# sapienta-ai/general-motion-retargeting

Measured on AMD Instinct MI355X. Metric: retargeted frames/sec (whole node) + max joint-angle err vs CPU ref, G1 29-DoF, higher is better.
Workload: dtype f64

## Files before the change

general_motion_retargeting_amd/csrc/gmr_ik.hip:

```cpp
#include <hip/hip_runtime.h>
#include <math.h>
#include <stdint.h>

#include "../../include/gmr_hip.h"
#include "gmr_device_math.h"
#include "gmr_ik_layout.h"
#include "gmr_ik_prof.h"

namespace gmr {

template <int NW>
__device__ __forceinline__ void wsync() {
  if (NW == 1) __syncthreads();
  else __builtin_amdgcn_fence(__ATOMIC_SEQ_CST, "workgroup");
}
#define WSYNC() wsync<NW>()

#ifndef GMR_IK_MIN_WAVES
#define GMR_IK_MIN_WAVES 1
#endif
enum { QP_DENSE = 0, QP_TREE_SMALL = 1, QP_TREE = 2 };
enum { CMD_BUILD = 1, CMD_EXIT = 2, CMD_JBODY = 3 };

__device__ __forceinline__ double readlane_d(double v, int src) {
  int lo = __builtin_amdgcn_readlane(__double2loint(v), src);
  int hi = __builtin_amdgcn_readlane(__double2hiint(v), src);
  return __hiloint2double(hi, lo);
}

__device__ __forceinline__ double bpermute_d(int addr, double v) {
  int lo = __builtin_amdgcn_ds_bpermute(addr, __double2loint(v));
  int hi = __builtin_amdgcn_ds_bpermute(addr, __double2hiint(v));
  return __hiloint2double(hi, lo);
}

__device__ __forceinline__ double dot6(const double* a, const double* b) {
  return a[0] * b[0] + a[1] * b[1] + a[2] * b[2] + a[3] * b[3] + a[4] * b[4] + a[5] * b[5];
}

}
#include "gmr_ik_tree.h"
namespace gmr {

struct FkLane {
  int dep, hinge, src[IK_MAX_HOPS];
  d4 bq; d3 bp, ax;
};

template <class LT>
__device__ __forceinline__ FkLane fk_lane(const LT& L, const double* sm, const short* hop, const short* depth,
                                          const short* body_hinge, int lane) {
  FkLane F;
  const int b = lane < L.nb ? lane : 0;
  F.dep = lane < L.nb ? depth[b] : 0;
  F.hinge = lane < L.nb ? body_hinge[b] : -1;
#pragma unroll
  for (int r = 0; r < IK_MAX_HOPS; r++) F.src[r] = r < L.nhop ? 4 * hop[r * L.o.cap.nb + b] : 0;
  const double* bq = sm + L.o.body_quat + 4 * b;
  const double* bp = sm + L.o.body_pos + 3 * b;
  const double* ax = sm + L.o.axis + 3 * b;
  F.bq = d4{bq[0], bq[1], bq[2], bq[3]};
  F.bp = d3{bp[0], bp[1], bp[2]};
  F.ax = d3{ax[0], ax[1], ax[2]};
  return F;
}

template <int NW, class LT>
__device__ __forceinline__ void fk_wave(const LT& L, double* sm, const FkLane& F, int lane, Prof& pr) {
  lane = fresh_lane(lane);
  PROF_BEGIN(pr);
  const int nb = L.nb;
  double* q = sm + L.o.q;
  d3 pos = {0, 0, 0};
  d4 quat = {1, 0, 0, 0};
  const int dep = F.dep;
  if (lane < nb) {
    if (lane == 0) {
      quat = qnormalize(d4{q[3], q[4], q[5], q[6]});
      q[3] = quat.w; q[4] = quat.x; q[5] = quat.y; q[6] = quat.z;
      pos = d3{q[0], q[1], q[2]};
    } else {
      quat = F.bq;
      pos = F.bp;
      if (F.hinge >= 0) {
        const double* sc = sm + L.o.hsc + 2 * F.hinge;
        const double s = sc[0], c = sc[1];
        quat = qmul(quat, d4{c, F.ax.x * s, F.ax.y * s, F.ax.z * s});
      }
    }
  }
#pragma unroll
  for (int r = 0; r < IK_MAX_HOPS; r++) {
    if (r >= L.nhop) break;
    const int src = F.src[r];
    const d3 pa = {bpermute_d(src, pos.x), bpermute_d(src, pos.y), bpermute_d(src, pos.z)};
    const d4 qa = {bpermute_d(src, quat.w), bpermute_d(src, quat.x), bpermute_d(src, quat.y), bpermute_d(src, quat.z)};
    if (NW > 1) __builtin_amdgcn_s_waitcnt(0xc07f);
    if (lane < nb && dep >= (1 << r)) {
      pos = pa + qrot(qa, pos);
      quat = qmul(qa, quat);
    }
  }
  if (lane < nb) {
    quat = qnormalize(quat);
    double* o = sm + L.o.xa + 7 * lane;
    o[0] = pos.x; o[1] = pos.y; o[2] = pos.z; o[3] = quat.w; o[4] = quat.x; o[5] = quat.y; o[6] = quat.z;
    if (F.hinge >= 0) {
      d3 aw = qrot(quat, F.ax);
      double* xa = sm + L.o.xaxis + 3 * lane;
      xa[0] = aw.x; xa[1] = aw.y; xa[2] = aw.z;
    }
  }
  WSYNC();
  PROF_END(pr, PH_FK);
}

template <int NW, class LT>
__device__ __forceinline__ double errors_wave(const LT& L, double* sm, const short* task_body,
                                              const short* task_human, int K, int lane, Prof& pr) {
  lane = fresh_lane(lane);
  PROF_BEGIN(pr);
  double ss = 0.0;
  if (lane < K) {
    int b = task_body[lane], h = task_human[lane];
    const double* x = sm + L.o.xa + 7 * b;
    const double* tg = sm + L.o.tgt + 7 * h;
    double e[6], aux[5];
    se3_log_rel5(d3{x[0], x[1], x[2]}, d4{x[3], x[4], x[5], x[6]}, d3{tg[0], tg[1], tg[2]},
                 d4{tg[3], tg[4], tg[5], tg[6]}, e, aux);
    double* eo = sm + L.o.e + 6 * lane;
#pragma unroll
    for (int r = 0; r < 6; r++) { eo[r] = e[r]; ss += e[r] * e[r]; }
    double* ao = sm + L.o.eaux + 5 * lane;
#pragma unroll
    for (int r = 0; r < 5; r++) ao[r] = aux[r];
  }
  ss = row0_sum(ss);
  WSYNC();
  PROF_END(pr, PH_ERR);
  return sqrt(ss);
}

struct StageTabs {
  const short* task_body; const short* task_human; const short* pair_task; const short* pair_dof;
  const short* pair_index; const uint2* items;
};

template <int NW, class LT>
__device__ __forceinline__ double jlog_phase(const LT& L, double* sm, int stage, double lm_damping, int lane,
                                             Prof& pr) {
  lane = fresh_lane(lane);
  PROF_BEGIN(pr);
  const int K = L.K[stage];
  const double* wpos = sm + L.o.wpos[stage];
  const double* wrot = sm + L.o.wrot[stage];
  double mu = 0.0;
  const int k = lane & 15, j = lane >> 4;
  if (NW > 1) {
    if (lane < K) {
      const double* e = sm + L.o.e + 6 * lane;
      double ee[6];
#pragma unroll
      for (int r = 0; r < 6; r++) ee[r] = e[r];
      const double* ax = sm + L.o.eaux + 5 * lane;
      const double aux[5] = {ax[0], ax[1], ax[2], ax[3], ax[4]};
      double coef[8];
      se3_jlinv_coef5(ee, aux, coef);
      double* co = sm + L.o.M + 18 * lane;
#pragma unroll
      for (int r = 0; r < 8; r++) co[r] = coef[r];
      const double wp = wpos[lane], wr = wrot[lane];
      double* we = sm + L.o.we + 6 * lane;
#pragma unroll
      for (int r = 0; r < 6; r++) {
        double v = (r < 3 ? wp : wr) * ee[r];
        we[r] = v;
        mu += v * v;
      }
    }
  } else if (k < K && j < 3) {
    const double* e = sm + L.o.e + 6 * k;
    double ee[6];
#pragma unroll
    for (int r = 0; r < 6; r++) ee[r] = e[r];
    const double* ax = sm + L.o.eaux + 5 * k;
    const double aux[5] = {ax[0], ax[1], ax[2], ax[3], ax[4]};
    double Ac[3], Bc[3];
    se3_jlinv_col5(ee, aux, j, Ac, Bc);
    double* M = sm + L.o.M + 18 * k + j;
#pragma unroll
    for (int i = 0; i < 3; i++) { M[3 * i] = -Ac[i]; M[9 + 3 * i] = -Bc[i]; }
    if (j == 0) {
      double wp = wpos[k], wr = wrot[k];
      double* we = sm + L.o.we + 6 * k;
#pragma unroll
      for (int r = 0; r < 6; r++) {
        double v = (r < 3 ? wp : wr) * ee[r];
        we[r] = v;
        mu += v * v;
      }
    }
  }
  mu = lm_damping * row0_sum(mu);
  WSYNC();
  PROF_END(pr, PH_JLOG);
  return mu;
}

template <class LT>
__device__ __forceinline__ void pairs_phase(const LT& L, double* sm, int stage, const StageTabs& tb,
                                            const short* hinge_body, int vlane, int nvl) {
  const int P = L.P[stage];
  const double* wpos = sm + L.o.wpos[stage];
  const double* wrot = sm + L.o.wrot[stage];
  double* Jw = sm + L.o.Jw;
  double* cpart = sm + L.o.cpart;
  const double* X = sm + L.o.xa;
  for (int p = vlane; p < P; p += nvl) {
    const unsigned info = (unsigned short)tb.pair_task[p];
    const int k = info & 15u, dof = (info >> 4) & 63u, b = info >> 10;
    const int c = tb.pair_dof[p];
    d3 pb = {X[7 * b], X[7 * b + 1], X[7 * b + 2]};
    d4 qb = {X[7 * b + 3], X[7 * b + 4], X[7 * b + 5], X[7 * b + 6]};
    d3 lin, ang;
    if (dof < 3) {
      lin = d3{dof == 0 ? 1.0 : 0.0, dof == 1 ? 1.0 : 0.0, dof == 2 ? 1.0 : 0.0};
      ang = d3{0.0, 0.0, 0.0};
    } else if (dof < 6) {
      d4 q0 = {X[3], X[4], X[5], X[6]};
      int a = dof - 3;
      ang = qrot(q0, d3{a == 0 ? 1.0 : 0.0, a == 1 ? 1.0 : 0.0, a == 2 ? 1.0 : 0.0});
      lin = cross(ang, pb - d3{X[0], X[1], X[2]});
    } else {
// ... 290 lines not shown
    PROF_END(hp, PH_CVEC);
    PROF_BEGIN(hp);
    hacc_phase(L, sm, stage, tb, diag, (wave - 1) * 64 + lane, first);
    PROF_END(hp, PH_HACC);
    PROF_BEGIN(hp);
    __syncthreads();
    PROF_END(hp, PH_JLOG);
    if (QP == QP_TREE_SMALL) (void)solve_qp_tree<7, 9, false, true>(L, sm, const_cast<uint32_t*>(sw), si, wave, lane, bs, hp, rows_s);
    else (void)solve_qp_tree<8, 10, false, false>(L, sm, const_cast<uint32_t*>(sw), si, wave, lane, bs, hp, rows_l);
  }
}

template <int NVP, int NW, class LT>
__device__ __forceinline__ int solve_qp_regs(const LT& L, double* sm, int lane, int& st, Prof& pr) {
  constexpr int LDK = NVP + 1;
  const int n = L.nv, ldh = L.o.ldh;
  const double* H = sm + L.o.H;
  double* Kt = sm + L.o.Kt;
  const bool act = lane < n;
  const bool row = lane < NVP;
  const double lo = act ? (sm + L.o.lo)[lane] : 0.0, hi = act ? (sm + L.o.hi)[lane] : 0.0;
  const double ci = act ? (sm + L.o.c)[lane] : 0.0;
  const double* Hrow = H + (act ? lane : 0) * ldh;
  if (!act || (st < 0 && !(lo > -INFINITY)) || (st > 0 && !(hi < INFINITY))) st = 0;
  const double dual_tol = 1e-13 * (1.0 + rows3_max(fabs(ci)));
  const double ptol_lo = 1e-12 * (1.0 + fabs(lo)), ptol_hi = 1e-12 * (1.0 + fabs(hi));
  int pcount = 3, ninf_best = NVP + 1;
  for (int it = 0; it < 100; it++) {
    PROF_BEGIN(pr);
    PROF_COUNT(pr, PH_NFACT);
    const unsigned long long fixedm = __ballot(act && st != 0);
    const double xfix = st < 0 ? lo : (st > 0 ? hi : 0.0);
    double rhs = act ? (st != 0 ? xfix : -ci) : 0.0;
    {
      unsigned long long m = fixedm;
      while (m) {
        int j = __ffsll((long long)m) - 1;
        m &= m - 1;
        double xj = readlane_d(xfix, j);
        if (act && st == 0) rhs -= Hrow[j] * xj;
      }
    }
    const bool self_fixed = (st != 0) || !act;
    double r[NVP];
#pragma unroll
    for (int k = 0; k < NVP; k++) {
      const bool kfixed = (k >= n) || ((fixedm >> k) & 1ull);
      double h = (act && k < n && k <= lane) ? Hrow[k] : 0.0;
      double v = (self_fixed || kfixed) ? 0.0 : h;
      if (k == lane && self_fixed) v = 1.0;
      r[k] = v;
    }
    PROF_END(pr, PH_KBUILD);
    PROF_BEGIN(pr);
    double mydinv = 1.0;
    bool bad = false;
#pragma unroll
    for (int j = 0; j < NVP; j++) {
      double dj = readlane_d(r[j], j);
      bad = bad || !(dj > 0.0);
      double dinv = fast_rsqrt(dj);
      double l = r[j] * dinv;
      r[j] = l;
      if (lane == j) mydinv = dinv;
#pragma unroll
      for (int k0 = j + 1; k0 < NVP; k0 += 4) {
        double lk[4];
#pragma unroll
        for (int u = 0; u < 4; u++) lk[u] = (k0 + u < NVP) ? readlane_d(l, k0 + u) : 0.0;
        __builtin_amdgcn_sched_barrier(0);
#pragma unroll
        for (int u = 0; u < 4; u++)
          if (k0 + u < NVP) r[k0 + u] = fma(-l, lk[u], r[k0 + u]);
        __builtin_amdgcn_sched_barrier(0);
      }
    }
    if (bad) return GMR_STATUS_QP_FAILED;
    PROF_END(pr, PH_CHOL);
    PROF_BEGIN(pr);
    double b = rhs;
#pragma unroll
    for (int j = 0; j < NVP; j++) {
      double yj = readlane_d(b * mydinv, j);
      double upd = fma(-r[j], yj, b);
      b = lane == j ? yj : (lane > j ? upd : b);
    }
    if (row) {
#pragma unroll
      for (int k = 0; k < NVP; k++) Kt[lane * LDK + k] = r[k];
    }
    WSYNC();
    double lt[NVP];
#pragma unroll
    for (int j = 0; j < NVP; j++) lt[j] = row ? Kt[j * LDK + lane] : 0.0;
#pragma unroll
    for (int j = NVP - 1; j >= 0; j--) {
      double xj = readlane_d(b * mydinv, j);
      double upd = fma(-lt[j], xj, b);
      b = lane == j ? xj : (lane < j ? upd : b);
    }
    double x = b;
    WSYNC();
    PROF_END(pr, PH_SUBST);
    PROF_BEGIN(pr);
    double g = 0.0;
    if (fixedm) {
      g = ci;
#pragma unroll
      for (int j = 0; j < NVP; j++) {
        double xj = readlane_d(x, j);
        if (j < n) g += (act ? Hrow[j] : 0.0) * xj;
      }
    }
    int newst = st;
    bool viol = false;
    if (act) {
      if (st == 0) {
        if (x < lo - ptol_lo) { viol = true; newst = -1; }
        else if (x > hi + ptol_hi) { viol = true; newst = 1; }
      } else if (st < 0) {
        if (g < -dual_tol) { viol = true; newst = 0; }
      } else {
        if (g > dual_tol) { viol = true; newst = 0; }
      }
    }
    const unsigned long long vm = __ballot(viol);
    PROF_END(pr, PH_MULT);
    if (vm == 0ull) {
      if (act) (sm + L.o.x)[lane] = fmin(fmax(x, lo), hi);
      WSYNC();
      return GMR_STATUS_OK;
    }
    const int ninf = __popcll(vm);
    if (ninf < ninf_best) { ninf_best = ninf; pcount = 3; st = newst; }
    else if (pcount > 0) { pcount--; st = newst; }
    else {
      int top = 63 - __clzll((long long)vm);
      if (lane == top) st = newst;
    }
  }
  return GMR_STATUS_QP_MAXITER;
}

template <class LT>
__device__ __forceinline__ void hinge_sincos(const LT& L, double* sm, int lane) {
  if (lane >= 6 && lane < L.nv) {
    double s, c;
    sincos_small(0.5 * (sm + L.o.q)[7 + lane - 6], &s, &c);
    double* sc = sm + L.o.hsc + 2 * (lane - 6);
    sc[0] = s; sc[1] = c;
  }
}

template <int NW, class LT>
__device__ __forceinline__ void integrate_wave(const LT& L, double* sm, double dt, int lane, Prof& pr) {
  lane = fresh_lane(lane);
  PROF_BEGIN(pr);
  double* q = sm + L.o.q;
  const double* dq = sm + L.o.x;
  const bool base = lane == 0, hinge = lane >= 6 && lane < L.nv;
  double half = 0.0, inv = 0.0;
  bool rotate = false;
  if (base) {
    q[0] += dq[0]; q[1] += dq[1]; q[2] += dq[2];
    const double n2 = dq[3] * dq[3] + dq[4] * dq[4] + dq[5] * dq[5];
    rotate = n2 >= 1e-30 * dt * dt;
    if (rotate) { inv = fast_rsqrt(n2); half = 0.5 * (n2 * inv); }
  } else if (hinge) {
    const double th = q[7 + lane - 6] + dq[lane];
    q[7 + lane - 6] = th;
    half = 0.5 * th;
  }
  double s, c;
  sincos_small(half, &s, &c);
  if (base) {
    d4 quat = qnormalize(d4{q[3], q[4], q[5], q[6]});
    if (rotate) quat = qmul(quat, d4{c, dq[3] * inv * s, dq[4] * inv * s, dq[5] * inv * s});
    q[3] = quat.w; q[4] = quat.x; q[5] = quat.y; q[6] = quat.z;
  } else if (hinge) {
    double* sc = sm + L.o.hsc + 2 * (lane - 6);
    sc[0] = s; sc[1] = c;
  }
  WSYNC();
  PROF_END(pr, PH_INTEG);
}

template <int NW, class LT>
__device__ __forceinline__ void preprocess_wave(const LT& L, double* sm, const short* is_foot, int human_root,
                                                double ground_offset, int flags, int lane, Prof& pr) {
  lane = fresh_lane(lane);
  PROF_BEGIN(pr);
  const double* raw = sm + L.o.raw;
  double* tgt = sm + L.o.tgt;
  double z = INFINITY;
  d3 p = {0, 0, 0};
  d4 uq = {1, 0, 0, 0};
  const bool on = lane < L.nhum;
  if (on) {
    const double* in = raw + 7 * lane;
    const double* rp = raw + 7 * human_root;
    const double* sc = sm + L.o.scale;
    double sr = sc[human_root];
    d3 srp = {sr * rp[0], sr * rp[1], sr * rp[2]};
    if (lane == human_root) p = srp;
    else {
      double s = sc[lane];
      p = d3{(in[0] - rp[0]) * s + srp.x, (in[1] - rp[1]) * s + srp.y, (in[2] - rp[2]) * s + srp.z};
    }
    const double* qo = sm + L.o.quat_off + 4 * lane;
    const double* po = sm + L.o.pos_off + 3 * lane;
    d4 q = qnormalize(d4{in[3], in[4], in[5], in[6]});
    uq = qnormalize(qmul(q, qnormalize(d4{qo[0], qo[1], qo[2], qo[3]})));
    p = p + qrot(uq, d3{po[0], po[1], po[2]});
    if (is_foot[lane] && p.x == p.x) z = p.z;
  }
  if (flags & GMR_FLAG_OFFSET_TO_GROUND) {
    double lowest = row0_min(z);
    p.z = p.z - lowest + ground_offset;
  }
  if (on) {
    double* o = tgt + 7 * lane;
    o[0] = p.x; o[1] = p.y; o[2] = p.z; o[3] = uq.w; o[4] = uq.x; o[5] = uq.y; o[6] = uq.z;
  }
  WSYNC();
  PROF_END(pr, PH_PRE);
}

template <int NVP, int NW, int QP>
__global__ __launch_bounds__(64 * NW, GMR_IK_MIN_WAVES) void ik_streams_kernel(const uint4* __restrict__ image, IkLay<NVP, NW> L, IkParams P,
                                                             int S, int T, const double* __restrict__ q0,
                                                             const double* __restrict__ human,
                                                             const int32_t* __restrict__ len, int flags,
                                                             double* __restrict__ q_out,
                                                             int32_t* __restrict__ nsolve,
                                                             int32_t* __restrict__ status,
                                                             double* __restrict__ tgt_out,
                                                             double* __restrict__ err_out,
                                                             unsigned long long* __restrict__ prof_out) {
  extern __shared__ __align__(16) double smem[];
  const int wave = threadIdx.x >> 6;
  const int lane = threadIdx.x & 63;
  const int s = blockIdx.x;
  if (s >= S) return;
  double* sm = smem;
  Prof pr;
#ifdef GMR_IK_PROFILE
  for (int i = 0; i < PH_COUNT; i++) pr.acc[i] = 0;
  const unsigned long long k_t0 = __builtin_amdgcn_s_memtime(), k_r0 = __builtin_amdgcn_s_memrealtime();
#endif
  short* si = reinterpret_cast<short*>(smem + L.o.n_double);
  uint32_t* sw = reinterpret_cast<uint32_t*>(si + L.o.n_short);
  int* ctl = reinterpret_cast<int*>(sw + L.o.w_ctl);
  short* hop = si + L.o.i_hop;
  short* depth = si + L.o.i_depth;
  short* body_hinge = si + L.o.i_body_hinge;
  short* hinge_body = si + L.o.i_hinge_body;
  short* limited = si + L.o.i_limited;
  short* is_foot = si + L.o.i_is_foot;

  const int nv = L.nv, nq = L.nq, nhum = L.nhum;
  {
    uint4* dst = reinterpret_cast<uint4*>(smem);
    const int n16 = (L.smem_bytes + 15) >> 4;
    for (int i = threadIdx.x; i < n16; i += 64 * NW) dst[i] = image[i];
  }
  __syncthreads();
  if (NW > 1 && wave > 0) {
    helper_loop<NW, QP>(L, sm, sw, si, hinge_body, ctl, wave, lane, pr);
#ifdef GMR_IK_PROFILE
    if (wave == 1 && lane == 0 && prof_out)
      for (int i = 0; i < PH_COUNT; i++) prof_out[((size_t)S + s) * PH_COUNT + i] = pr.acc[i];
#endif
    return;
  }
  const double* prm = sm + L.o.params;
  const int max_iter = P.max_iter, human_root = P.human_root;
  const int use0 = P.use0, use1 = P.use1;

  for (int i = lane; i < nq; i += 64) (sm + L.o.q)[i] = q0[(size_t)s * nq + i];
  WSYNC();
  hinge_sincos(L, sm, lane);
  WSYNC();
  const FkLane fkc = fk_lane(L, sm, hop, depth, body_hinge, lane);
  int pk_main[2];
#pragma unroll
  for (int st = 0; st < 2; st++) pk_main[st] = (unsigned short)(si + L.o.i_pair_task[st])[lane] & 15u;
  fk_wave<NW>(L, sm, fkc, lane, pr);

  const int Ts = len ? min(len[s], T) : T;
  const size_t fstride = (size_t)nhum * 7;
  const double* hs = human + (size_t)s * T * fstride;
  int stat = GMR_STATUS_OK;
  int qp_state = 0;
  TreeState tree_state = {0ull, 0ull};
  const TreeRows<16> rows_s = (NW > 1 && QP == QP_TREE_SMALL) ? tree_rows<7, 9, false>(L, si, 0, lane) : TreeRows<16>{};
  const TreeRows<18> rows_l = (NW > 1 && QP != QP_TREE_SMALL) ? tree_rows<8, 10, false>(L, si, 0, lane) : TreeRows<18>{};
  const TreeRows<16> rows_r = (NW == 1 && QP == QP_TREE_SMALL) ? tree_rows<7, 9, true>(L, si, 0, lane) : TreeRows<16>{};
  int h_stage = -1;
  int epoch = 0;
  double r0 = 0.0, r1 = 0.0;
  if (Ts > 0) {
    if (lane < (int)fstride) r0 = hs[lane];
    if (lane + 64 < (int)fstride) r1 = hs[lane + 64];
  }
  for (int t = 0; t < Ts; t++) {
    if (lane < (int)fstride) (sm + L.o.raw)[lane] = r0;
    if (lane + 64 < (int)fstride) (sm + L.o.raw)[lane + 64] = r1;
    if (t + 1 < Ts) {
      const double* nx = hs + (size_t)(t + 1) * fstride;
      if (lane < (int)fstride) r0 = nx[lane];
      if (lane + 64 < (int)fstride) r1 = nx[lane + 64];
    }
    WSYNC();
    int ns0 = 0, ns1 = 0;
    const size_t f = (size_t)s * T + t;
    if (stat == GMR_STATUS_OK) {
      preprocess_wave<NW>(L, sm, is_foot, human_root, prm[4], flags, lane, pr);
      if (tgt_out)
        for (int i = lane; i < (int)fstride; i += 64) tgt_out[f * fstride + i] = (sm + L.o.tgt)[i];
      double last_E = -1.0;
      for (int stage = 0; stage < 2; stage++) {
        if (!(stage == 0 ? use0 : use1) || (flags & GMR_FLAG_EVAL_ONLY)) continue;
        const StageTabs tb = {si + L.o.i_task_body[stage], si + L.o.i_task_human[stage], si + L.o.i_pair_task[stage],
                              si + L.o.i_pair_dof[stage], si + L.o.i_pair_index[stage],
                              reinterpret_cast<const uint2*>(NW == 1 ? reinterpret_cast<const uint32_t*>(image) + L.g_items[stage]
                                                                     : sw + L.w_items[stage])};
        const int K = L.K[stage];
        if (h_stage != stage) {
          for (int i = lane; i < nv * L.o.ldh; i += 64) (sm + L.o.H)[i] = 0.0;
          h_stage = stage;
          WSYNC();
        }
        if (NW > 1 && !(stage == 1 && (use1 & 4) && last_E >= 0.0)) {
          if (lane == 0) { int* c = ctl + 2 * (epoch & 1); c[0] = CMD_JBODY; c[1] = stage; }
          epoch++;
          __syncthreads();
        }
        double curr = (stage == 1 && (use1 & 2) && last_E >= 0.0) ? last_E
                                                                 : errors_wave<NW>(L, sm, tb.task_body, tb.task_human, K, lane, pr);
        int nsol = 0, num_iter = 0;
        for (;;) {
          build_qp_main<NW>(L, sm, stage, tb, hinge_body, limited, ctl, epoch, prm[0], prm[1], prm[3], lane, pk_main[stage], pr);
          PROF_COUNT(pr, PH_NSOLVE);
          int rc;
          if (NW > 1) {
            rc = QP == QP_TREE_SMALL ? solve_qp_tree<7, 9, false, true>(L, sm, sw, si, 0, lane, tree_state, pr, rows_s)
                                     : solve_qp_tree<8, 10, false, false>(L, sm, sw, si, 0, lane, tree_state, pr, rows_l);
          } else if (QP == QP_TREE_SMALL) {
            rc = solve_qp_tree<7, 9, true, true>(L, sm, sw, si, 0, lane, tree_state, pr, rows_r);
          } else {
            rc = solve_qp_regs<NVP, NW>(L, sm, lane, qp_state, pr);
          }
          if (rc != GMR_STATUS_OK) { stat = rc; break; }
          integrate_wave<NW>(L, sm, prm[5], lane, pr);
          fk_wave<NW>(L, sm, fkc, lane, pr);
          if (NW > 1) {
            if (lane == 0) { int* c = ctl + 2 * (epoch & 1); c[0] = CMD_JBODY; c[1] = stage; }
            epoch++;
            __syncthreads();
          }
          double next = errors_wave<NW>(L, sm, tb.task_body, tb.task_human, K, lane, pr);
          last_E = next;
          nsol++;
          if (nsol > 1) num_iter++;
          if (!(curr - next > prm[2] && num_iter < max_iter)) break;
          curr = next;
        }
        if (stage == 0) ns0 = nsol; else ns1 = nsol;
        if (stat != GMR_STATUS_OK) break;
      }
    }
    if (err_out && stat == GMR_STATUS_OK) {
      for (int stage = 0; stage < 2; stage++) {
        double E = 0.0;
        if (stage == 0 ? use0 : use1)
          E = errors_wave<NW>(L, sm, si + L.o.i_task_body[stage], si + L.o.i_task_human[stage], L.K[stage], lane, pr);
        if (lane == 0) err_out[2 * f + stage] = E;
      }
    }
    for (int i = lane; i < nq; i += 64) q_out[f * nq + i] = (sm + L.o.q)[i];
    if (lane == 0) { nsolve[2 * f] = ns0; nsolve[2 * f + 1] = ns1; }
    WSYNC();
  }
  if (lane == 0) status[s] = stat;
  if (NW > 1) {
    if (lane == 0) ctl[2 * (epoch & 1)] = CMD_EXIT;
    __syncthreads();
  }
#ifdef GMR_IK_PROFILE
  pr.acc[PH_TICKS] = __builtin_amdgcn_s_memtime() - k_t0;
  pr.acc[PH_REALTIME] = __builtin_amdgcn_s_memrealtime() - k_r0;
  if (lane == 0 && prof_out)
    for (int i = 0; i < PH_COUNT; i++) prof_out[(size_t)s * PH_COUNT + i] = pr.acc[i];
#else
  (void)prof_out;
#endif
}

}

template <int NVP, int NW, int QP>
static hipError_t launch_nvp(const uint4* d_image, const gmr::IkLayout* L, const gmr::IkParams* P, int S, int T,
                             const double* d_q0, const double* d_human,
                             const int32_t* d_len, int flags, double* d_q_out, int32_t* d_nsolve, int32_t* d_status,
                             double* d_tgt_out, double* d_err_out, hipStream_t stream, unsigned long long* d_prof) {
  hipLaunchKernelGGL((gmr::ik_streams_kernel<NVP, NW, QP>), dim3(S), dim3(64 * NW), L->smem_bytes, stream, d_image,
                     gmr::IkLay<NVP, NW>(static_cast<const gmr::IkDims&>(*L)), *P, S, T, d_q0, d_human, d_len, flags, d_q_out, d_nsolve, d_status,
                     d_tgt_out, d_err_out, d_prof);
  return hipGetLastError();
}

#define GMR_ARGS d_image, L, P, S, T, d_q0, d_human, d_len, flags, d_q_out, d_nsolve, d_status, d_tgt_out, d_err_out, stream, d_prof
#define GMR_DISPATCH(NVP_)                                                                             \
  case NVP_:                                                                                           \
    if (L->nw == 1) return L->tree_small ? launch_nvp<NVP_, 1, gmr::QP_TREE_SMALL>(GMR_ARGS)           \
                                         : launch_nvp<NVP_, 1, gmr::QP_DENSE>(GMR_ARGS);               \
    return L->tree_small ? launch_nvp<NVP_, 4, gmr::QP_TREE_SMALL>(GMR_ARGS)                           \
                         : launch_nvp<NVP_, 4, gmr::QP_TREE>(GMR_ARGS);

extern "C" hipError_t gmr_launch_ik_streams(const uint4* d_image, const gmr::IkLayout* L, const gmr::IkParams* P,
                                            int S, int T, const double* d_q0, const double* d_human,
                                            const int32_t* d_len, int flags, double* d_q_out, int32_t* d_nsolve,
                                            int32_t* d_status, double* d_tgt_out, double* d_err_out,
                                            hipStream_t stream, unsigned long long* d_prof) {
  if (S <= 0 || T <= 0) return hipSuccess;
  switch (L->nvp) {
    GMR_DISPATCH(28)
    GMR_DISPATCH(32)
    GMR_DISPATCH(36)
    GMR_DISPATCH(48)
    default: return hipErrorInvalidValue;
  }
}

template <int NVP>
static const void* kernel_of(int nw, int tree_small) {
  if (nw == 1) return tree_small ? reinterpret_cast<const void*>(gmr::ik_streams_kernel<NVP, 1, gmr::QP_TREE_SMALL>)
                                 : reinterpret_cast<const void*>(gmr::ik_streams_kernel<NVP, 1, gmr::QP_DENSE>);
  return tree_small ? reinterpret_cast<const void*>(gmr::ik_streams_kernel<NVP, 4, gmr::QP_TREE_SMALL>)
                    : reinterpret_cast<const void*>(gmr::ik_streams_kernel<NVP, 4, gmr::QP_TREE>);
}

extern "C" hipError_t gmr_ik_set_max_smem(int nvp, int nw, int tree_small, int bytes) {
  const void* f = nullptr;
  switch (nvp) {
    case 28: f = kernel_of<28>(nw, tree_small); break;
    case 32: f = kernel_of<32>(nw, tree_small); break;
    case 36: f = kernel_of<36>(nw, tree_small); break;
    case 48: f = kernel_of<48>(nw, tree_small); break;
    default: return hipErrorInvalidValue;
  }
  return hipFuncSetAttribute(f, hipFuncAttributeMaxDynamicSharedMemorySize, bytes);
}
```

general_motion_retargeting_amd/csrc/gmr_ik_layout.h:

```cpp
#pragma once
#include <stdint.h>

#include <algorithm>
#include <cstring>
#include <vector>

#include "../../include/gmr_types.h"

namespace gmr {

constexpr int IK_MAX_ZERO = 64;
constexpr int IK_MAX_HOPS = 5;

struct IkCaps { int nb, nh, k, p, nhum; };
constexpr IkCaps ik_caps(int nvp) {
  return nvp == 28 ? IkCaps{34, 22, 16, 160, 16}
       : nvp == 32 ? IkCaps{34, 26, 16, 160, 16}
       : nvp == 36 ? IkCaps{40, 30, 16, 160, 16}
                   : IkCaps{GMR_MAX_BODIES, GMR_MAX_HINGES, GMR_MAX_TASKS, GMR_MAX_PAIRS, GMR_MAX_HUMAN};
}

struct IkOffsets {
  IkCaps cap;
  int nvp;
  int ldh;
  int body_pos, body_quat, axis, range_lo, range_hi, scale, pos_off, quat_off;
  int wpos[2], wrot[2];
  int q, xa, xb, xaxis, raw, tgt, e, eaux, we, M, Jw, cpart, H, Kt, c, x, lo, hi, scal, tr_spart, tr_rpart, tr_gpart;
  int params;
  int hsc;
  int n_double;
  int i_hop, i_depth, i_body_hinge, i_hinge_body, i_limited, i_is_foot, i_tree_limb, i_tree_trunk;
  int i_task_body[2], i_task_human[2], i_pair_task[2], i_pair_dof[2], i_pair_index[2];
  int n_short;
  int w_ctl, w_tr_mask, w_tr_cnt, w_zero, w_items0;
  int fixed_bytes;
};

constexpr int ik_max(int a, int b) { return a > b ? a : b; }

constexpr IkOffsets ik_offsets(int nvp, int nw) {
  IkOffsets L{};
  const IkCaps cp = ik_caps(nvp);
  L.cap = cp;
  L.nvp = nvp;
  L.ldh = nvp + 1;
  int o = 0;
  L.body_pos = o; o += 3 * cp.nb; L.body_quat = o; o += 4 * cp.nb; L.axis = o; o += 3 * cp.nb;
  L.range_lo = o; o += cp.nh; L.range_hi = o; o += cp.nh;
  L.params = o; o += 6;
  L.scale = o; o += cp.nhum; L.pos_off = o; o += 3 * cp.nhum; L.quat_off = o; o += 4 * cp.nhum;
  for (int s = 0; s < 2; s++) { L.wpos[s] = o; o += cp.k; L.wrot[s] = o; o += cp.k; }
  L.q = o; o += 7 + cp.nh + 1;
  L.hsc = o; o += 2 * cp.nh;
  L.xa = o; o += 7 * cp.nb + 1;
  L.xaxis = o; o += 3 * cp.nb;
  L.tgt = o; o += 7 * cp.nhum + 1;
  L.e = o; o += 6 * cp.k; L.eaux = o; o += 5 * cp.k; L.we = o; o += 6 * cp.k;
  L.M = o; o += ik_max(18 * cp.k, 7 * cp.nhum + 1);
  L.raw = L.M;
  if (o & 1) o++;
  L.Jw = o; o += ik_max(6 * (cp.p + 1), 7 * cp.nb + 1);
  L.cpart = o; o += cp.p + 1;
  L.xb = L.Jw;
  {
    const int rows_scr = 4 * 16 * 19;
    const int need = nw == 4 ? ik_max(nvp * (nvp + 1), 4 * 18 * 19) : ik_max(nvp * (nvp + 1), rows_scr + 440);
    const int have = o - L.e;
    if (have < need) o += need - have;
    L.Kt = L.e;
    if (nw != 4) { L.tr_spart = L.Kt + rows_scr; L.tr_rpart = L.tr_spart + 400; }
  }
  if (o & 1) o++;
  L.H = o; o += nvp * L.ldh + 2;
  L.c = o; o += nvp; L.x = o; o += nvp; L.lo = o; o += nvp; L.hi = o; o += nvp; L.scal = o; o += 2;
  if (nw == 4) { L.tr_spart = o; o += 4 * 10 * 10; L.tr_rpart = o; o += 4 * 10; L.tr_gpart = o; o += 4 * 10; }
  if (o & 1) o++;
  L.n_double = o;
  int i = 0;
  L.i_hop = i; i += IK_MAX_HOPS * cp.nb; L.i_depth = i; i += cp.nb; L.i_body_hinge = i; i += cp.nb;
  L.i_hinge_body = i; i += cp.nh; L.i_limited = i; i += cp.nh; L.i_is_foot = i; i += cp.nhum;
  L.i_tree_limb = i; i += 4 * 8; L.i_tree_trunk = i; i += 10;
  for (int s = 0; s < 2; s++) {
    L.i_task_body[s] = i; i += cp.k; L.i_task_human[s] = i; i += cp.k;
    L.i_pair_task[s] = i; i += cp.p; L.i_pair_dof[s] = i; i += cp.p;
    L.i_pair_index[s] = i; i += cp.k * nvp;
  }
  L.n_short = (i + 7) / 8 * 8;
  int w = 0;
  L.w_ctl = w; w += 4;
  L.w_tr_mask = w; w += 16;
  L.w_tr_cnt = w; w += 4;
  L.w_zero = w; w += 2 * IK_MAX_ZERO;
  if (w % 4) w += 4 - w % 4;
  L.w_items0 = w;
  L.fixed_bytes = L.n_double * 8 + L.n_short * 2 + w * 4;
  return L;
}

struct IkDims {
  int nb, nh, nq, nv, nhum, nhop, tree_ok;
  int tree_small;
  int K[2], P[2], ntrip[2], nlanes, pair_lanes;
  int atomic_lanes[2], nzero[2];
  int w_items[2];
  int g_items[2];
  int smem_bytes;
};

struct IkLayout : IkDims {
  int nvp, nw, maxd, tree_nt, nitem[2], image_bytes;
  IkOffsets o;
};

template <int NVP, int NW>
struct IkLay : IkDims {
  static constexpr IkOffsets o = ik_offsets(NVP, NW);
  IkLay() = default;
  explicit IkLay(const IkDims& d) : IkDims(d) {}
};

inline int ik_padded_nv(int nv) {
  if (nv <= 28) return 28;
  if (nv <= 32) return 32;
  if (nv <= 36) return 36;
  if (nv <= 48) return 48;
  return -1;
}

inline int ik_size_class(const gmr_model_t& m, const gmr_taskset_t& ts) {
  for (int nvp : {28, 32, 36, 48}) {
    const IkCaps c = ik_caps(nvp);
    if (m.nv <= nvp && m.nbody <= c.nb && m.nhinge <= c.nh && ts.nhuman <= c.nhum && ts.ntask[0] <= c.k &&
        ts.ntask[1] <= c.k && ts.npair[0] <= c.p && ts.npair[1] <= c.p)
      return nvp;
  }
  return -1;
}

constexpr uint64_t ik_item_nop(int zero_row) { return (uint64_t)(48u * (uint32_t)zero_row) * 0x10001ull; }

struct IkSchedule {
  int nlanes;
  int pair_lanes;
  std::vector<uint64_t> items[2];
  std::vector<int> istart[2];
  int ntrip[2];
  int npaired[2];
  int atomic_lanes[2];
  std::vector<int> zero_off[2];
  std::vector<uint64_t> padded[2];
};

inline IkSchedule make_ik_schedule(const gmr_model_t& m, const gmr_taskset_t& ts, int nlanes, int ldh, int zero_row) {
  IkSchedule sch;
  const uint64_t NOP = ik_item_nop(zero_row);
  sch.nlanes = nlanes;
  sch.pair_lanes = nlanes > 64 ? 64 : 0;
  const int nv = m.nv;
  for (int s = 0; s < 2; s++) {
    std::vector<std::vector<uint32_t>> terms((size_t)nv * nv);
    for (int k = 0; k < ts.ntask[s]; k++) {
      int c0 = ts.task_col0[s][k], n = ts.task_ncol[s][k];
      for (int a = 0; a < n; a++)
        for (int b = 0; b <= a; b++) {
          int da = ts.pair_dof[s][c0 + a], db = ts.pair_dof[s][c0 + b];
          terms[(size_t)da * nv + db].push_back(48u * (uint32_t)(c0 + a) | ((48u * (uint32_t)(c0 + b)) << 16));
        }
    }
    struct Ent { int da, db, w, t0, t1, atomic; };
    auto dest = [&](const Ent& e) {
      return (uint64_t)((uint32_t)(8 * (e.da * ldh + e.db)) | ((uint32_t)(8 * (e.db * ldh + e.da)) << 15) |
                        (e.da == e.db && e.t0 == 0 ? 1u << 30 : 0u)) << 32;
    };
    std::vector<Ent> ents;
    for (int da = 0; da < nv; da++)
      for (int db = 0; db <= da; db++) {
        int w = (int)terms[(size_t)da * nv + db].size();
        if (w > 0 || da == db) ents.push_back({da, db, w, 0, w, 0});
      }
    std::stable_sort(ents.begin(), ents.end(), [](const Ent& x, const Ent& y) { return x.w > y.w; });
    std::vector<std::vector<Ent>> per_lane(nlanes);
    std::vector<Ent> pair_ents;
    std::vector<Ent> singles;
    sch.atomic_lanes[s] = 0;
    sch.zero_off[s].clear();
    if (sch.pair_lanes) {
      const int npair = sch.pair_lanes / 2;
      size_t nheavy = 0;
      while (nheavy < ents.size() && ents[nheavy].w > 8) nheavy++;
      size_t next = 0;
      if (nheavy > 0 && 2 * (int)nheavy <= npair && 2 * (int)nheavy <= IK_MAX_ZERO) {
        for (; next < nheavy; next++) {
          const Ent& e = ents[next];
          const int h = (e.w + 1) / 2;
          pair_ents.push_back({e.da, e.db, h, 0, h, 1});
          pair_ents.push_back({e.da, e.db, e.w - h, h, e.w, 1});
          sch.zero_off[s].push_back(8 * (e.da * ldh + e.db));
          if (e.da != e.db) sch.zero_off[s].push_back(8 * (e.db * ldh + e.da));
        }
        sch.atomic_lanes[s] = 2 * (int)pair_ents.size();
      }
      for (; next < ents.size() && (int)pair_ents.size() < npair && ents[next].w >= 4; next++) pair_ents.push_back(ents[next]);
      for (; next < ents.size(); next++) singles.push_back(ents[next]);
    } else {
      singles = ents;
    }
    {
      const int l0 = sch.pair_lanes, nl1 = nlanes - l0;
      int total = 0;
      for (const Ent& e : singles) total += std::max(e.w, 1);
      for (int cap = std::max(4, ((total + nl1 - 1) / nl1 + 3) & ~3);; cap += 4) {
        for (int l = l0; l < nlanes; l++) per_lane[l].clear();
        std::vector<int> load(nlanes, 0);
        bool fits = true;
        for (const Ent& e : singles) {
          int lane = -1;
          for (int l = l0; l < nlanes && lane < 0; l++) if (load[l] + std::max(e.w, 1) <= cap) lane = l;
          if (lane < 0) { fits = false; break; }
          per_lane[lane].push_back(e);
          load[lane] += std::max(e.w, 1);
        }
        if (fits) break;
      }
    }
    sch.npaired[s] = (int)pair_ents.size();
    sch.items[s].clear();
    sch.istart[s].assign(nlanes + 1, 0);
    for (int l = 0; l < nlanes; l++) {
// ... 226 lines not shown
```

general_motion_retargeting_amd/csrc/gmr_ik_tree.h:

```cpp
#pragma once

namespace gmr {

constexpr int TR_MAX_NL = 8;
constexpr int TR_MAX_NT = 10;

struct TreeState { unsigned long long lower, upper; };

template <int TR_NV>
struct TreeRows { int dof; int cdof[TR_NV]; };

template <int TR_NL, int TR_NT, bool ROWS, class LT>
__device__ __forceinline__ TreeRows<TR_NL + TR_NT> tree_rows(const LT& L, const short* si, int wave_in, int lane_in) {
  const int wave = ROWS ? (lane_in >> 4) : wave_in, lane = ROWS ? (lane_in & 15) : lane_in;
  const short* limb = si + L.o.i_tree_limb + wave * TR_MAX_NL;
  const short* trunk = si + L.o.i_tree_trunk;
  TreeRows<TR_NL + TR_NT> R;
  R.dof = lane < TR_NL ? limb[lane] : (lane < TR_NL + TR_NT ? trunk[lane - TR_NL] : -1);
#pragma unroll
  for (int m = 0; m < TR_NL; m++) R.cdof[m] = limb[m];
#pragma unroll
  for (int u = 0; u < TR_NT; u++) R.cdof[TR_NL + u] = trunk[u];
  return R;
}

template <int TR_NL, int TR_NT, bool ROWS, bool DPPB, class LT>
__device__ __forceinline__ int solve_qp_tree(const LT& L, double* sm, uint32_t* sw, const short* si, int wave_in,
                                             int lane_in, TreeState& bs, Prof& pr, const TreeRows<TR_NL + TR_NT>& rows) {
  constexpr int TR_NV = TR_NL + TR_NT;
  static_assert(!ROWS || TR_NV <= 16, "a limb's local matrix must fit one 16-lane row");
  const int wave = ROWS ? (lane_in >> 4) : wave_in;
  const int lane0 = ROWS ? (lane_in & 15) : lane_in;
#define TR_ROW()                                                                                   \
  const int lane = fresh_lane(lane0);                                                              \
  const bool is_limb = lane < TR_NL, is_trunk = lane >= TR_NL && lane < TR_NV;                     \
  const int a = lane, t = lane - TR_NL;                                                            \
  (void)is_limb; (void)is_trunk; (void)a; (void)t;
  const int lane = lane0;
  static_assert(!DPPB || TR_NV <= 16, "DPP row broadcasts need the local matrix in one 16-lane row");
#define TR_BCAST(v, k) ((ROWS || DPPB) ? row_bcast_d((v), (k)) : readlane_d((v), (k)))
#define TR_SYNC() do { if (ROWS) __builtin_amdgcn_fence(__ATOMIC_SEQ_CST, "workgroup"); else __syncthreads(); } while (0)
  const int n = L.nv, ldh = L.o.ldh;
  const double* H = sm + L.o.H;
  double* xs = sm + L.o.x;
  const double* los = sm + L.o.lo;
  const double* his = sm + L.o.hi;
  double* Spart = sm + L.o.tr_spart;
  double* rpart = sm + L.o.tr_rpart;
  double* gpart = sm + L.o.tr_gpart;
  unsigned long long* vset = reinterpret_cast<unsigned long long*>(sw + L.o.w_tr_mask);

  const bool is_limb = lane < TR_NL, is_trunk = lane >= TR_NL && lane < TR_NV;
  const int a = lane, t = lane - TR_NL;
  const int dof = rows.dof;
  const bool row = dof >= 0;
  const bool own = row && (is_limb || wave == 0);
  const double lo = row ? los[dof] : 0.0, hi = row ? his[dof] : 0.0;
  const double ci = row ? (sm + L.o.c)[dof] : 0.0;
  const double* Hrow = H + (row ? dof : 0) * ldh;
  double dual_tol = -1.0;
  const double ptol_lo = 1e-12 * (1.0 + fabs(lo)), ptol_hi = 1e-12 * (1.0 + fabs(hi));
  const int* cdof = rows.cdof;

  double h[TR_NV];
#pragma unroll
  for (int m = 0; m < TR_NV; m++) h[m] = Hrow[cdof[m] >= 0 ? cdof[m] : 0];

  int pcount = 3, ninf_best = 65;
  for (int it = 0; it < 100; it++) {
    PROF_COUNT(pr, PH_NFACT);
    PROF_BEGIN(pr);
    const unsigned long long fixedm = bs.lower | bs.upper;
    const bool self_fixed = !row || ((fixedm >> dof) & 1ull);
    const double xfix = !row ? 0.0 : (((bs.lower >> dof) & 1ull) ? lo : (((bs.upper >> dof) & 1ull) ? hi : 0.0));
    const unsigned long long fixed_lanes = __ballot(self_fixed);
    const unsigned colmask = (ROWS ? (unsigned)(fixed_lanes >> (16 * wave)) : (unsigned)fixed_lanes) & ((1u << TR_NV) - 1u);
    double r[TR_NV];
#pragma unroll
    for (int m = 0; m < TR_NV; m++) r[m] = 0.0;
    double rhs0, b;
    {
    TR_ROW()
#pragma unroll
    for (int m = 0; m < TR_NL; m++) {
      const bool cfixed = (colmask >> m) & 1u;
      const bool keep = row && !self_fixed && !cfixed;
      double v = keep ? h[m] : 0.0;
      if (is_limb && m == a && (self_fixed || cfixed)) v = 1.0;
      r[m] = v;
    }
#pragma unroll
    for (int u = 0; u < TR_NT; u++) {
      const bool cfixed = (colmask >> (TR_NL + u)) & 1u;
      r[TR_NL + u] = (is_limb && row && !self_fixed && !cfixed) ? h[TR_NL + u] : 0.0;
    }
    rhs0 = row ? (self_fixed ? xfix : -ci) : 0.0;
    double bshare = 0.0;
    if (fixedm != 0ull) {
      double sl0 = 0.0, sl1 = 0.0, st0 = 0.0, st1 = 0.0;
#pragma unroll
      for (int m = 0; m < TR_NL; m++) {
        const double xf = TR_BCAST(xfix, m);
        if (m & 1) sl1 = fma(h[m], xf, sl1); else sl0 = fma(h[m], xf, sl0);
      }
#pragma unroll
      for (int u = 0; u < TR_NT; u++) {
        const double xf = TR_BCAST(xfix, TR_NL + u);
        if (u & 1) st1 = fma(h[TR_NL + u], xf, st1); else st0 = fma(h[TR_NL + u], xf, st0);
      }
      const double sl = sl0 + sl1, st = st0 + st1;
      if (row && !self_fixed) {
        rhs0 = is_limb ? (rhs0 - st) - sl : rhs0 - st;
        bshare = -sl;
      }
    }
    b = is_limb ? rhs0 : (is_trunk ? bshare : 0.0);
    }
    PROF_END(pr, PH_KBUILD);
    PROF_BEGIN(pr);
    double mydinv = 1.0;
    bool bad = false;
    double dp = TR_BCAST(r[0], 0);
    double dinv = fast_rsqrt(dp);
#pragma unroll
    for (int p = 0; p < TR_NL; p++) {
      const int lane = fresh_lane(lane0);
      bad = bad || !(dp > 0.0);
      const double rs = r[p] * dinv;
      double l = lane > p ? rs : 0.0;
      if (lane == p) mydinv = dinv;
      double dinv_next = 1.0;
      if (p + 1 < TR_NL) {
        r[p + 1] = fma(-l, TR_BCAST(l, p + 1), r[p + 1]);
        dp = TR_BCAST(r[p + 1], p + 1);
        dinv_next = fast_rsqrt(dp);
      }
      const double yp = TR_BCAST(b, p) * dinv;
      b = fma(-l, yp, b);
#pragma unroll
      for (int k = (p + 1 < TR_NL ? p + 2 : p + 1); k < TR_NV; k++) r[k] = fma(-l, TR_BCAST(l, k), r[k]);
      dinv = dinv_next;
    }
    if (fresh_lane(lane0) < TR_NL) b *= mydinv;
    double ltl[TR_NL], yl[TR_NT];
    {
      TR_ROW()
#pragma unroll
      for (int m = 0; m < TR_NL; m++) ltl[m] = (is_limb && m > a) ? r[m] * mydinv : 0.0;
#pragma unroll
      for (int u = 0; u < TR_NT; u++) yl[u] = r[TR_NL + u] * mydinv;
    }
    PROF_END(pr, PH_CHOL);
    PROF_BEGIN(pr);
    unsigned long long* vcur = vset + 4 * (it & 1);
    {
    TR_ROW()
    if (is_trunk) {
#pragma unroll
      for (int u = 0; u < TR_NT; u++) Spart[(wave * TR_MAX_NT + t) * TR_MAX_NT + u] = r[TR_NL + u];
      rpart[wave * TR_MAX_NT + t] = b;
    }
    if (lane == 0 && bad) atomicOr(&vcur[3], 1ull);
    TR_SYNC();
    if (wave == 0 && lane < 4) vset[4 * ((it + 1) & 1) + lane] = 0ull;
    }
    PROF_END(pr, PH_SUBST);
    PROF_BEGIN(pr);
    double bt = 0.0;
    bool tbad = false;
    {
      double s[TR_NT];
#pragma unroll
      for (int u = 0; u < TR_NT; u++) s[u] = 0.0;
      {
        TR_ROW()
        const int tt = is_trunk ? t : 0;
        double hv[TR_NT], sp[TR_NT];
#pragma unroll
        for (int u = 0; u < TR_NT; u++) {
          hv[u] = h[TR_NL + u];
          const double* q0 = Spart + tt * TR_MAX_NT + u;
          sp[u] = (q0[0] + q0[TR_MAX_NT * TR_MAX_NT]) + (q0[2 * TR_MAX_NT * TR_MAX_NT] + q0[3 * TR_MAX_NT * TR_MAX_NT]);
        }
        const double rp = (rpart[tt] + rpart[TR_MAX_NT + tt]) + (rpart[2 * TR_MAX_NT + tt] + rpart[3 * TR_MAX_NT + tt]);
        const bool live = is_trunk && row && !self_fixed;
#pragma unroll
        for (int u = 0; u < TR_NT; u++) {
          const bool cfixed = (colmask >> (TR_NL + u)) & 1u;
          double v = (live && !cfixed) ? hv[u] + sp[u] : 0.0;
          if (is_trunk && u == t && !(live && !cfixed)) v = 1.0;
          s[u] = v;
        }
        bt = is_trunk ? (live ? rhs0 + rp : rhs0) : 0.0;
      }
      double tdinv = 1.0;
      double dq = TR_BCAST(s[0], TR_NL);
      double dinv = fast_rsqrt(dq);
#pragma unroll
      for (int q = 0; q < TR_NT; q++) {
        const int t = fresh_lane(lane0) - TR_NL;
        tbad = tbad || !(dq > 0.0);
        const double ss = s[q] * dinv;
        double l = t > q ? ss : 0.0;
        if (t == q) tdinv = dinv;
        double dinv_next = 1.0;
        if (q + 1 < TR_NT) {
          s[q + 1] = fma(-l, TR_BCAST(l, TR_NL + q + 1), s[q + 1]);
          dq = TR_BCAST(s[q + 1], TR_NL + q + 1);
          dinv_next = fast_rsqrt(dq);
        }
        const double yq = TR_BCAST(bt, TR_NL + q) * dinv;
        bt = fma(-l, yq, bt);
#pragma unroll
        for (int k = q + 2; k < TR_NT; k++) s[k] = fma(-l, TR_BCAST(l, TR_NL + k), s[k]);
        dinv = dinv_next;
      }
      double lt[TR_NT];
      {
        TR_ROW()
#pragma unroll
        for (int q = 0; q < TR_NT; q++) lt[q] = (is_trunk && q > t) ? s[q] * tdinv : 0.0;
      }
      bt *= tdinv;
#pragma unroll
      for (int q = TR_NT - 1; q >= 0; q--) {
        const double xq = TR_BCAST(bt * tdinv, TR_NL + q);
        bt = fma(-lt[q], xq, bt);
      }
      bt *= tdinv;
    }
    PROF_END(pr, PH_RATIO);
    PROF_BEGIN(pr);
    double x = bt;
    {
      double bb = b;
      {
        TR_ROW()
#pragma unroll
        for (int u = 0; u < TR_NT; u++) {
          const double xt = TR_BCAST(bt, TR_NL + u);
          if (is_limb) bb = fma(-yl[u], xt, bb);
        }
      }
#pragma unroll
      for (int p = TR_NL - 1; p >= 0; p--) {
        const double xp = TR_BCAST(bb * mydinv, p);
        bb = fma(-ltl[p], xp, bb);
      }
      if (fresh_lane(lane0) < TR_NL) x = bb * mydinv;
    }
    double pl = 0.0, pt = 0.0;
    bool trunk_fixed = false;
    if (fixedm != 0ull) {
      if (dual_tol < 0.0) {
        const int li = fresh_lane(lane_in);
        dual_tol = 1e-13 * (1.0 + rows3_max(li < n ? fabs((sm + L.o.c)[li]) : 0.0));
      }
      if (ROWS) {
        if (own) xs[dof] = x;
        TR_SYNC();
      } else {
        double pl1 = 0.0, pt1 = 0.0;
#pragma unroll
        for (int m = 0; m < TR_NL; m++) {
          const double xm = TR_BCAST(x, m);
          if (m & 1) pl1 = fma(h[m], xm, pl1); else pl = fma(h[m], xm, pl);
        }
#pragma unroll
        for (int u = 0; u < TR_NT; u++) {
          const double xu = TR_BCAST(x, TR_NL + u);
          if (u & 1) pt1 = fma(h[TR_NL + u], xu, pt1); else pt = fma(h[TR_NL + u], xu, pt);
        }
        pl += pl1; pt += pt1;
        TR_ROW()
        trunk_fixed = __any(is_trunk && row && self_fixed);
        if (trunk_fixed) {
          if (is_trunk) gpart[wave * TR_MAX_NT + t] = pl;
          TR_SYNC();
        }
      }
    }
    PROF_END(pr, PH_MULT);
    PROF_BEGIN(pr);
    int newst = 0;
    if (own) {
      if (!self_fixed) {
        if (x < lo - ptol_lo) newst = 1;
        else if (x > hi + ptol_hi) newst = 2;
      } else {
        double g;
        if (ROWS) {
          double g0 = ci, g1 = 0.0;
          double g2 = 0.0, g3 = 0.0;
          int j = 0;
          for (; j + 7 < n; j += 8) {
            const double h0 = Hrow[j], h1 = Hrow[j + 1], h2 = Hrow[j + 2], h3 = Hrow[j + 3], h4 = Hrow[j + 4], h5 = Hrow[j + 5],
                         h6 = Hrow[j + 6], h7 = Hrow[j + 7];
            const double x0 = xs[j], x1 = xs[j + 1], x2 = xs[j + 2], x3 = xs[j + 3], x4 = xs[j + 4], x5 = xs[j + 5],
                         x6 = xs[j + 6], x7 = xs[j + 7];
            g0 = fma(h0, x0, g0); g1 = fma(h1, x1, g1); g2 = fma(h2, x2, g2); g3 = fma(h3, x3, g3);
            g0 = fma(h4, x4, g0); g1 = fma(h5, x5, g1); g2 = fma(h6, x6, g2); g3 = fma(h7, x7, g3);
          }
          for (; j < n; j++) g0 = fma(Hrow[j], xs[j], g0);
          g = (g0 + g1) + (g2 + g3);
        } else {
          const int lane = fresh_lane(lane0);
          g = ci + (pl + pt);
          if (lane >= TR_NL) {
            const double* gp = gpart + (lane - TR_NL);
            g = (ci + pt) + ((gp[0] + gp[TR_MAX_NT]) + (gp[2 * TR_MAX_NT] + gp[3 * TR_MAX_NT]));
          }
        }
        const bool at_lower = (bs.lower >> dof) & 1ull;
        if (at_lower ? g < -dual_tol : g > dual_tol) newst = 3;
      }
    }
    if (newst != 0) atomicOr(&vcur[newst - 1], 1ull << dof);
    if (fresh_lane(lane0) == 0 && tbad) atomicOr(&vcur[3], 1ull);
    const bool early = !ROWS || fixedm == 0ull;
    if (early && own && newst == 0) xs[dof] = fmin(fmax(x, lo), hi);
    TR_SYNC();
    PROF_END(pr, PH_IO);
    const unsigned long long to_lo = vcur[0], to_up = vcur[1], rel = vcur[2];
    if (vcur[3]) return GMR_STATUS_QP_FAILED;
    const unsigned long long all = to_lo | to_up | rel;
    if (all == 0ull) {
      if (!early) {
        if (own) xs[dof] = fmin(fmax(x, lo), hi);
        TR_SYNC();
      }
      return GMR_STATUS_OK;
    }
    const int total = __popcll(all);
    unsigned long long sel = all;
    if (total < ninf_best) { ninf_best = total; pcount = 3; }
    else if (pcount > 0) pcount--;
    else sel = 1ull << (63 - __clzll((long long)all));
    bs.lower = (bs.lower & ~(rel & sel)) | (to_lo & sel);
    bs.upper = (bs.upper & ~(rel & sel)) | (to_up & sel);
  }
  return GMR_STATUS_QP_MAXITER;
#undef TR_BCAST
#undef TR_SYNC
#undef TR_ROW
}

}
```

Measured before the change: 845,200.

## Fuse integration step into tree QP solver final iteration for multi-wave path

For the multi-wave tree QP path, each solver iteration now speculatively computes the integrated hinge angles, hinge sin/cos, and base pose from its candidate solution. The results are committed when the active set converges, which removes the separate integrate_wave pass and its synchronization. The base pose is staged in a new shared buffer (qbase) that fk_wave reads instead of renormalizing q. In exchange, every QP iteration now does sincos and quaternion work even though only the last one is used, and the layout and state handling become more complex.

```diff
diff --git a/general_motion_retargeting_amd/csrc/gmr_ik.hip b/general_motion_retargeting_amd/csrc/gmr_ik.hip
--- a/general_motion_retargeting_amd/csrc/gmr_ik.hip
+++ b/general_motion_retargeting_amd/csrc/gmr_ik.hip
@@ -76,9 +76,16 @@
   const int dep = F.dep;
   if (lane < nb) {
     if (lane == 0) {
-      quat = qnormalize(d4{q[3], q[4], q[5], q[6]});
-      q[3] = quat.w; q[4] = quat.x; q[5] = quat.y; q[6] = quat.z;
-      pos = d3{q[0], q[1], q[2]};
+      if (NW > 1) {
+        const double* st = sm + L.o.qbase;
+        pos = d3{st[0], st[1], st[2]};
+        quat = d4{st[3], st[4], st[5], st[6]};
+        q[0] = pos.x; q[1] = pos.y; q[2] = pos.z; q[3] = quat.w; q[4] = quat.x; q[5] = quat.y; q[6] = quat.z;
+      } else {
+        quat = qnormalize(d4{q[3], q[4], q[5], q[6]});
+        q[3] = quat.w; q[4] = quat.x; q[5] = quat.y; q[6] = quat.z;
+        pos = d3{q[0], q[1], q[2]};
+      }
     } else {
       quat = F.bq;
       pos = F.bp;
@@ -675,6 +682,17 @@
   }
 }
 
+template <class LT>
+__device__ __forceinline__ void stage_base(const LT& L, double* sm, int lane) {
+  if (lane == 0) {
+    const double* q = sm + L.o.q;
+    const d4 quat = qnormalize(d4{q[3], q[4], q[5], q[6]});
+    double* st = sm + L.o.qbase;
+    st[0] = q[0]; st[1] = q[1]; st[2] = q[2];
+    st[3] = quat.w; st[4] = quat.x; st[5] = quat.y; st[6] = quat.z;
+  }
+}
+
 template <int NW, class LT>
 __device__ __forceinline__ void integrate_wave(const LT& L, double* sm, double dt, int lane, Prof& pr) {
   lane = fresh_lane(lane);
@@ -803,6 +821,7 @@
   for (int i = lane; i < nq; i += 64) (sm + L.o.q)[i] = q0[(size_t)s * nq + i];
   WSYNC();
   hinge_sincos(L, sm, lane);
+  if (NW > 1) stage_base(L, sm, lane);
   WSYNC();
   const FkLane fkc = fk_lane(L, sm, hop, depth, body_hinge, lane);
   int pk_main[2];
@@ -875,7 +894,7 @@
             rc = solve_qp_regs<NVP, NW>(L, sm, lane, qp_state, pr);
           }
           if (rc != GMR_STATUS_OK) { stat = rc; break; }
-          integrate_wave<NW>(L, sm, prm[5], lane, pr);
+          if (NW == 1) integrate_wave<NW>(L, sm, prm[5], lane, pr);
           fk_wave<NW>(L, sm, fkc, lane, pr);
           if (NW > 1) {
             if (lane == 0) { int* c = ctl + 2 * (epoch & 1); c[0] = CMD_JBODY; c[1] = stage; }
diff --git a/general_motion_retargeting_amd/csrc/gmr_ik_layout.h b/general_motion_retargeting_amd/csrc/gmr_ik_layout.h
--- a/general_motion_retargeting_amd/csrc/gmr_ik_layout.h
+++ b/general_motion_retargeting_amd/csrc/gmr_ik_layout.h
@@ -35,6 +35,7 @@
   int n_short;
   int w_ctl, w_tr_mask, w_tr_cnt, w_zero, w_items0;
   int fixed_bytes;
+  int qbase;
 };
 
 constexpr int ik_max(int a, int b) { return a > b ? a : b; }
@@ -74,7 +75,7 @@
   if (o & 1) o++;
   L.H = o; o += nvp * L.ldh + 2;
   L.c = o; o += nvp; L.x = o; o += nvp; L.lo = o; o += nvp; L.hi = o; o += nvp; L.scal = o; o += 2;
-  if (nw == 4) { L.tr_spart = o; o += 4 * 10 * 10; L.tr_rpart = o; o += 4 * 10; L.tr_gpart = o; o += 4 * 10; }
+  if (nw == 4) { L.tr_spart = o; o += 4 * 10 * 10; L.tr_rpart = o; o += 4 * 10; L.tr_gpart = o; o += 4 * 10; L.qbase = o; o += 8; }
   if (o & 1) o++;
   L.n_double = o;
   int i = 0;
diff --git a/general_motion_retargeting_amd/csrc/gmr_ik_tree.h b/general_motion_retargeting_amd/csrc/gmr_ik_tree.h
--- a/general_motion_retargeting_amd/csrc/gmr_ik_tree.h
+++ b/general_motion_retargeting_amd/csrc/gmr_ik_tree.h
@@ -57,6 +57,16 @@
   const bool own = row && (is_limb || wave == 0);
   const double lo = row ? los[dof] : 0.0, hi = row ? his[dof] : 0.0;
   const double ci = row ? (sm + L.o.c)[dof] : 0.0;
+  const bool hinge_own = !ROWS && own && dof >= 6;
+  double* qs = sm + L.o.q;
+  const double qh = hinge_own ? qs[7 + dof - 6] : 0.0;
+  double qb[7] = {0.0, 0.0, 0.0, 1.0, 0.0, 0.0, 0.0};
+  double dt = 0.0;
+  if (!ROWS && wave == 0) {
+    dt = (sm + L.o.params)[5];
+#pragma unroll
+    for (int i = 0; i < 7; i++) qb[i] = qs[i];
+  }
   const double* Hrow = H + (row ? dof : 0) * ldh;
   double dual_tol = -1.0;
   const double ptol_lo = 1e-12 * (1.0 + fabs(lo)), ptol_hi = 1e-12 * (1.0 + fabs(hi));
@@ -318,7 +328,48 @@
     if (newst != 0) atomicOr(&vcur[newst - 1], 1ull << dof);
     if (fresh_lane(lane0) == 0 && tbad) atomicOr(&vcur[3], 1ull);
     const bool early = !ROWS || fixedm == 0ull;
-    if (early && own && newst == 0) xs[dof] = fmin(fmax(x, lo), hi);
+    double th = 0.0;
+    if (ROWS) {
+      if (early && own && newst == 0) xs[dof] = fmin(fmax(x, lo), hi);
+    } else {
+      PROF_END(pr, PH_IO);
+      PROF_BEGIN(pr);
+      const int lane = fresh_lane(lane0);
+      const double xc = fmin(fmax(x, lo), hi);
+      const bool keep = own && newst == 0;
+      if (keep) xs[dof] = xc;
+      th = qh + xc;
+      double half = 0.5 * th, inv = 0.0;
+      bool rotate = false;
+      double dq[6] = {0.0, 0.0, 0.0, 0.0, 0.0, 0.0};
+      if (wave == 0) {
+#pragma unroll
+        for (int i = 0; i < 6; i++) dq[i] = TR_BCAST(xc, TR_NL + i);
+        const double n2 = dq[3] * dq[3] + dq[4] * dq[4] + dq[5] * dq[5];
+        rotate = n2 >= 1e-30 * dt * dt;
+        double hb = 0.0;
+        if (rotate) { inv = fast_rsqrt(n2); hb = 0.5 * (n2 * inv); }
+        if (lane == TR_NL) half = hb;
+      }
+      double s, c;
+      sincos_small(half, &s, &c);
+      if (hinge_own && keep) {
+        double* sc = sm + L.o.hsc + 2 * (dof - 6);
+        sc[0] = s; sc[1] = c;
+      }
+      if (wave == 0) {
+        d4 quat = qnormalize(d4{qb[3], qb[4], qb[5], qb[6]});
+        if (rotate) quat = qmul(quat, d4{c, dq[3] * inv * s, dq[4] * inv * s, dq[5] * inv * s});
+        quat = qnormalize(quat);
+        if (lane == TR_NL) {
+          double* st = sm + L.o.qbase;
+          st[0] = qb[0] + dq[0]; st[1] = qb[1] + dq[1]; st[2] = qb[2] + dq[2];
+          st[3] = quat.w; st[4] = quat.x; st[5] = quat.y; st[6] = quat.z;
+        }
+      }
+      PROF_END(pr, PH_INTEG);
+      PROF_BEGIN(pr);
+    }
     TR_SYNC();
     PROF_END(pr, PH_IO);
     const unsigned long long to_lo = vcur[0], to_up = vcur[1], rel = vcur[2];
@@ -329,6 +380,7 @@
         if (own) xs[dof] = fmin(fmax(x, lo), hi);
         TR_SYNC();
       }
+      if (hinge_own) qs[7 + dof - 6] = th;
       return GMR_STATUS_OK;
     }
     const int total = __popcll(all);
```

Result: no change. 852,400 (median of 6 runs) (+0.8%).
